# POSTECH-CVLab/InstaOrder

Hardware: AMD Instinct MI355X
Metric: instance-pairs/sec (fwd+bwd) (higher is better)
Workload: dtype f32

## Files before the change

instaorder_amd/csrc/conv_igemm.hip:

```cpp
#include <string.h>
#include <stdlib.h>

#include "io_common.h"

namespace {

constexpr int kThreads = 256;

__device__ __forceinline__ f32x4 ld4(const float* p) { return *reinterpret_cast<const f32x4*>(p); }
template <typename T> __device__ __forceinline__ void pin(T& v) { asm volatile("" : "+v"(v)); }
__device__ __forceinline__ void st4(float* p, f32x4 v) { *reinterpret_cast<f32x4*>(p) = v; }

__device__ __forceinline__ int xcd_remap(int b, int nwg) {
    const int q = nwg >> 3, r = nwg & 7, x = b & 7, i = b >> 3;
    return (x < r ? x * (q + 1) : r * (q + 1) + (x - r) * q) + i;
}

__device__ __forceinline__ int sdiv(int n, float rd) { return (int)(((float)n + 0.5f) * rd); }
__device__ __forceinline__ int stem_kp(int wT, int cr) { return (wT * cr + 31) / 32 * 32; }
__device__ __forceinline__ int fdiv(int n, IoFastDiv f) {
    return f.shift < 0 ? n : (int)(__umulhi((unsigned)n, f.magic) >> f.shift);
}

typedef unsigned u32x4 __attribute__((ext_vector_type(4)));
// ... 1958 lines not shown
        read_frags(0, na, nb);
        __builtin_amdgcn_sched_barrier(0);
        mma12(3, fa, fb);
#pragma unroll
        for (int j = 0; j < 3; ++j) { fa[j] = na[j]; fb[j] = nb[j]; }
    }
    if (kt0 < kt1) {
#pragma unroll
        for (int gi = 0; gi < 3; ++gi) {
            f32x4 na[3], nb[3];
            read_frags(gi + 1, na, nb);
            mma12(gi, fa, fb);
#pragma unroll
            for (int j = 0; j < 3; ++j) { fa[j] = na[j]; fb[j] = nb[j]; }
        }
        mma12(3, fa, fb);
    }

    const size_t wrow = (size_t)g.wT * g.Ci;
    float* base = dst + (size_t)split * g.Co * wrow + (size_t)(g.r0 + g.rs * fr) * g.S * g.Ci + c0 + wn * 32 + (lane & 31);
#pragma unroll
    for (int r = 0; r < 16; ++r) {
        const int o = o0 + wm * 32 + (r & 3) + 8 * (r >> 2) + 4 * (lane >> 5);
        const float s12 = acc[1][r] + acc[2][r], s34 = acc[3][r] + acc[4][r];
        float* p = base + (size_t)o * wrow;
        p[0] = 0.25f * acc[0][r] - (1.0f / 6.0f) * s12 + (1.0f / 24.0f) * s34;
        p[g.Ci] = (1.0f / 6.0f) * (acc[2][r] - acc[1][r]) + (1.0f / 12.0f) * (acc[3][r] - acc[4][r]);
        p[2 * g.Ci] = (1.0f / 6.0f) * (s34 - s12) + acc[5][r];
    }
}



template <bool BWE, bool XF, bool HALO = false>
__global__ __launch_bounds__(256, 2) void conv_wino4_kernel(IoConvGeom g, const float* __restrict__ in,
                                                        const float* __restrict__ U, float* __restrict__ out, int ntn,
                                                        size_t in_bytes, unsigned u_bytes, size_t out_bytes,
                                                        float* __restrict__ st_mean, float* __restrict__ st_m2,
                                                        IoBwStats bw) {
    constexpr int BM = 256, BN = 64, BK = 16, LDT = 16, NF = 6;
    constexpr int AQ = HALO ? 96 : 64;
    extern __shared__ __attribute__((aligned(16))) float smem[];
    float* sA = smem;
    float* sB = smem + NF * AQ * LDT;
    const int tid = threadIdx.x, lane = tid & 63;
    const int wave = __builtin_amdgcn_readfirstlane(tid >> 6);
    const int wm = wave >> 1, wn = wave & 1;
    const int tile = xcd_remap(blockIdx.x, gridDim.x);
    const int mt = tile / ntn;
    const int m0 = mt * BM, n0 = (tile - mt * ntn) * BN;
    const int HoWo = g.Ho * g.Wo;
    const int nkc = g.Ci / BK, nk = 3 * nkc;
    const int n_lo = fdiv(m0, g.fd_howo);
    const __amdgpu_buffer_rsrc_t rs_in = make_rsrc_at(in, (size_t)n_lo * (size_t)(g.Hi * g.Wi) * (size_t)(g.Ci * 4), in_bytes);
    const __amdgpu_buffer_rsrc_t rs_u = make_rsrc(U, u_bytes);

    const int sr = tid >> 2, sc = tid & 3;
    unsigned arow, urow;
    int aho;
    bool aleft, aright;
    constexpr int NI = HALO ? 2 : 1;
    const int Q = g.Wo >> 2;
    const int ns = HALO ? (HoWo >= BM ? 1 : BM / HoWo) : 1;
    const int RS = HALO ? (64 / Q) / ns : 1;
    const int HB = (RS + 2) * Q, hq_n = ns * HB;
    unsigned hrow[NI];
    bool hvalid[NI], hleft[NI], hright[NI];
    const bool has2 = HALO && 64 + sr < hq_n;
    const bool wave_has2 = HALO && 64 + wave * 16 < hq_n;
    if constexpr (HALO) {
        const int rem0 = m0 - n_lo * HoWo;
        const int h0 = ns > 1 ? 0 : fdiv(rem0, g.fd_wo);
#pragma unroll
        for (int it = 0; it < NI; ++it) {
            const int hq = sr + 64 * it;
            const int sm = hq / HB, hl = hq - sm * HB;
            const int hr = hl / Q, cq = hl - hr * Q;
            const int hi = h0 - 1 + hr, wo = 4 * cq;
            hvalid[it] = (it == 0 || has2) && (unsigned)hi < (unsigned)g.Hi;
            hleft[it] = wo > 0;
            hright[it] = wo + 4 < g.Wi;
            hrow[it] = (unsigned)((((sm * g.Hi + hi) * g.Wi + wo) * g.Ci + sc * 4) * 4);
        }
        aho = 0; aleft = aright = false; arow = 0;
        urow = (unsigned)((n0 + sr) * g.Ci + sc * 4) * 4u;
    } else {
        const int m = m0 + 4 * sr;
        const int n = fdiv(m, g.fd_howo), rem = m - n * HoWo;
        const int ho = fdiv(rem, g.fd_wo), wo = rem - ho * g.Wo;
        aho = ho;
        aleft = wo > 0;
        aright = wo + 4 < g.Wi;
        arow = (unsigned)((((n - n_lo) * g.Hi + ho) * g.Wi + wo) * g.Ci + sc * 4) * 4u;
        urow = (unsigned)((n0 + sr) * g.Ci + sc * 4) * 4u;
    }
    const unsigned uplane = (unsigned)(g.Co * g.Ci) * 4u;
    const int xgrp = XF ? m0 / bw.in_Mg : 0;
    const __amdgpu_buffer_rsrc_t rs_xs = make_rsrc(XF ? (const void*)(bw.in_scale + (size_t)xgrp * g.Ci) : (const void*)U,
                                                   XF ? (unsigned)g.Ci * 4u : 0u);
    const __amdgpu_buffer_rsrc_t rs_xh = make_rsrc(XF ? (const void*)(bw.in_shift + (size_t)xgrp * g.Ci) : (const void*)U,
                                                   XF ? (unsigned)g.Ci * 4u : 0u);
    const __amdgpu_buffer_rsrc_t rs_xm = make_rsrc((XF && bw.in_mean) ? (const void*)(bw.in_mean + (size_t)xgrp * g.Ci)
                                                                      : (const void*)U,
                                                   (XF && bw.in_mean) ? (unsigned)g.Ci * 4u : 0u);
    f32x4 pa[6], pu[6], xm, xs, xh;
    f32x4 pa2[HALO ? 6 : 1];
    unsigned xok = 0, xok2 = 0;
    int th = 0, cc = 0;
    auto load_tile = [&]() {
        const unsigned uoff = (unsigned)(th * NF) * uplane + (unsigned)(cc * BK) * 4u;
        if constexpr (HALO) {
#pragma unroll
            for (int f = 0; f < NF; ++f) pu[f] = bld4(rs_u, urow + uoff + (unsigned)f * uplane);
            if (th != 0) return;
            if constexpr (XF) {
                const unsigned coff = (unsigned)(cc * BK + sc * 4) * 4u;
                xm = bld4(rs_xm, coff);
                xs = bld4(rs_xs, coff);
                xh = bld4(rs_xh, coff);
            }
            const unsigned aoff = (unsigned)((cc * BK - g.Ci) * 4);
            xok = xok2 = 0;
#pragma unroll
            for (int i = 0; i < 6; ++i) {
                const bool ok = hvalid[0] & (i == 0 ? hleft[0] : i == 5 ? hright[0] : true);
                xok |= ok ? (1u << i) : 0u;
                pa[i] = bld4(rs_in, ok ? hrow[0] + aoff + (unsigned)(i * g.Ci * 4) : kInvalidOff);
            }
            if (wave_has2) {
#pragma unroll
                for (int i = 0; i < 6; ++i) {
                    const bool ok = hvalid[NI - 1] & (i == 0 ? hleft[NI - 1] : i == 5 ? hright[NI - 1] : true);
                    xok2 |= ok ? (1u << i) : 0u;
                    pa2[i] = bld4(rs_in, ok ? hrow[NI - 1] + aoff + (unsigned)(i * g.Ci * 4) : kInvalidOff);
                }
            }
            return;
        }
        const int dh = g.dh0 + g.dhs * th;
        const unsigned aoff = (unsigned)(((dh * g.Wi - 1) * g.Ci + cc * BK) * 4);
        if constexpr (XF) {
            const unsigned coff = (unsigned)(cc * BK + sc * 4) * 4u;
            xm = bld4(rs_xm, coff);
            xs = bld4(rs_xs, coff);
            xh = bld4(rs_xh, coff);
        }
        const bool rowok = (unsigned)(aho + dh) < (unsigned)g.Hi;
        xok = 0;
#pragma unroll
        for (int i = 0; i < 6; ++i) {
            const bool ok = rowok & (i == 0 ? aleft : i == 5 ? aright : true);
            xok |= ok ? (1u << i) : 0u;
            pa[i] = bld4(rs_in, ok ? arow + aoff + (unsigned)(i * g.Ci * 4) : kInvalidOff);
        }
#pragma unroll
        for (int f = 0; f < NF; ++f) pu[f] = bld4(rs_u, urow + uoff + (unsigned)f * uplane);
    };
    auto advance = [&]() {
        if constexpr (HALO) {
            const bool wrap = th == 2;
            th = wrap ? 0 : th + 1;
            cc += wrap ? 1 : 0;
            return;
        }
        const int c1 = cc + 1;
        const bool wrap = c1 == nkc;
        cc = wrap ? 0 : c1;
        th += wrap ? 1 : 0;
    };
    auto xform_item = [&](f32x4 (&p)[6], unsigned okbits) {
        if constexpr (XF) {
#pragma unroll
            for (int i = 0; i < 6; ++i) {
                const bool ok = (okbits >> i) & 1u;
#pragma unroll
                for (int e = 0; e < 4; ++e) {
                    const float v = fmaxf(__builtin_fmaf(p[i][e] - xm[e], xs[e], xh[e]), 0.f);
                    p[i][e] = ok ? v : 0.f;
                }
            }
        }
        const f32x4 d0 = p[0], d1 = p[1], d2 = p[2], d3 = p[3], d4 = p[4], d5 = p[5];
        const f32x4 e42 = d4 - 4.f * d2, e31 = d3 - 4.f * d1, f42 = d4 - d2, f31 = d3 - d1;
        p[0] = 4.f * d0 - 5.f * d2 + d4;
        p[1] = e42 + e31;
        p[2] = e42 - e31;
        p[3] = f42 + 2.f * f31;
        p[4] = f42 - 2.f * f31;
        p[5] = 4.f * d1 - 5.f * d3 + d5;
    };
    auto xform_tile = [&]() {
        if constexpr (HALO) {
            if (th != 0) return;
            xform_item(pa, xok);
            if (wave_has2) xform_item(pa2, xok2);
            return;
        }
        xform_item(pa, xok);
    };
    const int swz = sc ^ ((sr >> 2) & 3);
    auto store_tile = [&]() {
        float* a = sA + sr * LDT + swz * 4;
        float* b = sB + sr * LDT + swz * 4;
        if constexpr (HALO) {
#pragma unroll
            for (int f = 0; f < NF; ++f) st4(b + f * 64 * LDT, pu[f]);
            if (th != 0) return;
#pragma unroll
            for (int f = 0; f < NF; ++f) st4(a + f * AQ * LDT, pa[f]);
            if (has2) {
#pragma unroll
                for (int f = 0; f < NF; ++f) st4(a + (f * AQ + 64) * LDT, pa2[f]);
            }
            return;
        }
#pragma unroll
        for (int f = 0; f < NF; ++f) {
            st4(a + f * 64 * LDT, pa[f]);
            st4(b + f * 64 * LDT, pu[f]);
        }
    };

    f32x16 acc[NF];
#pragma unroll
    for (int f = 0; f < NF; ++f)
#pragma unroll
        for (int r = 0; r < 16; ++r) acc[f][r] = 0.f;

    const int frow = lane & 31;
    const int b_base = (wn * 32 + frow) * LDT;
    const int fsw = (frow >> 2) & 3;
    int arow_cur = wm * 32 + frow;
    const int arow_lane = HALO ? (wm * 32 + frow) + ((wm * 32 + frow) / (RS * Q)) * 2 * Q : 0;
    auto set_hoff = [&](int thc) {
        if constexpr (HALO) arow_cur = arow_lane + (1 + g.dh0 + g.dhs * thc) * Q;
    };
    auto read_frags = [&](int gi, f32x4 (&a)[3], f32x4 (&b)[3]) {
        const int cl = (gi >> 1) * 2 + (lane >> 5);
        const int chunk = cl ^ fsw;
        const int chunk_a = HALO ? (cl ^ ((arow_cur >> 2) & 3)) : chunk;
        const int f0 = (gi & 1) * 3;
#pragma unroll
        for (int j = 0; j < 3; ++j) {
            a[j] = ld4(sA + ((f0 + j) * AQ + arow_cur) * LDT + chunk_a * 4);
            b[j] = ld4(sB + (f0 + j) * 64 * LDT + b_base + chunk * 4);
        }
    };
    auto mma12 = [&](int gi, const f32x4 (&a)[3], const f32x4 (&b)[3]) {
        const int f0 = (gi & 1) * 3;
#pragma unroll
        for (int tt = 0; tt < 4; ++tt)
#pragma unroll
            for (int j = 0; j < 3; ++j)
                acc[f0 + j] = __builtin_amdgcn_mfma_f32_32x32x2f32(a[j][tt], b[j][tt], acc[f0 + j], 0, 0, 0);
    };

    f32x4 fa[3], fb[3];
    load_tile();
    xform_tile();
    store_tile();
    __syncthreads();
    int thc = 0;
    set_hoff(0);
    read_frags(0, fa, fb);
    for (int kt = 0; kt + 1 < nk; ++kt) {
        advance();
#pragma unroll
        for (int gi = 0; gi < 3; ++gi) {
            f32x4 na[3], nb[3];
            read_frags(gi + 1, na, nb);
            mma12(gi, fa, fb);
#pragma unroll
            for (int j = 0; j < 3; ++j) { fa[j] = na[j]; fb[j] = nb[j]; }
            if (gi == 0) {
                load_tile();
                __builtin_amdgcn_sched_barrier(0);
            }
            if (gi == 1) xform_tile();
        }
        __builtin_amdgcn_sched_barrier(0);
#pragma unroll
        for (int j = 0; j < 3; ++j) { pin(fa[j]); pin(fb[j]); }
        __syncthreads();
        store_tile();
        __syncthreads();
        thc = thc == 2 ? 0 : thc + 1;
        set_hoff(thc);
        f32x4 na[3], nb[3];
        read_frags(0, na, nb);
        __builtin_amdgcn_sched_barrier(0);
        mma12(3, fa, fb);
#pragma unroll
        for (int j = 0; j < 3; ++j) { fa[j] = na[j]; fb[j] = nb[j]; }
    }
#pragma unroll
    for (int gi = 0; gi < 3; ++gi) {
        f32x4 na[3], nb[3];
        read_frags(gi + 1, na, nb);
        mma12(gi, fa, fb);
#pragma unroll
        for (int j = 0; j < 3; ++j) { fa[j] = na[j]; fb[j] = nb[j]; }
    }
    mma12(3, fa, fb);

#pragma unroll
    for (int r = 0; r < 16; ++r) {
        const float s12 = acc[1][r] + acc[2][r], d12 = acc[1][r] - acc[2][r];
        const float s34 = acc[3][r] + acc[4][r], d34 = acc[3][r] - acc[4][r];
        const float y0 = acc[0][r] + s12 + s34, y3 = d12 + 8.f * d34 + acc[5][r];
        acc[1][r] = d12 + 2.f * d34;
        acc[2][r] = s12 + 4.f * s34;
        acc[0][r] = y0;
        acc[3][r] = y3;
    }
    const int st = 2 * mt + wm;
    const int co = n0 + wn * 32 + (lane & 31);
    if (st_mean) {
        float sum = 0.f;
#pragma unroll
        for (int i = 0; i < 4; ++i)
#pragma unroll
            for (int r = 0; r < 16; ++r) sum += acc[i][r];
        sum += __shfl_xor(sum, 32, 64);
        const float mean = sum * (1.0f / 128.0f);
        float m2 = 0.f;
#pragma unroll
        for (int i = 0; i < 4; ++i)
#pragma unroll
            for (int r = 0; r < 16; ++r) m2 += (acc[i][r] - mean) * (acc[i][r] - mean);
        m2 += __shfl_xor(m2, 32, 64);
        if (lane < 32) {
            st_mean[(size_t)st * g.Co + co] = mean;
            st_m2[(size_t)st * g.Co + co] = m2;
        }
    }
    const size_t out_base = (size_t)(m0 + wm * 128) * (size_t)(g.Co * 4);
// ... 20 lines not shown
                const float t = __builtin_fmaf(yv[r] - mu, sc_, sh_);
                float v = acc[i][r];
                if (bw.mscale) v = t > 0.f ? v : 0.f;
                s1 += v;
                s2 += v * ((yv[r] - mu) * rs);
                st_el_s<float>(v, rs_out, lane_off, so);
                st_el_s<float>(fmaxf(t, 0.f), rs_ao, lane_off, so);
            }
        }
        s1 += __shfl_xor(s1, 32, 64);
        s2 += __shfl_xor(s2, 32, 64);
        if (lane < 32) {
            bw.p1[(size_t)st * g.Co + co] = s1;
            bw.p2[(size_t)st * g.Co + co] = s2;
        }
    } else {
        const float bias = bw.bias ? bw.bias[co] : 0.f;
#pragma unroll
        for (int i = 0; i < 4; ++i)
#pragma unroll
            for (int r = 0; r < 16; ++r) {
                float v = acc[i][r];
                if (bw.bias) {
                    v += bias;
                    v = (bw.relu && v < 0.f) ? 0.f : v;
                }
                st_el_s<float>(v, rs_out, lane_off, (unsigned)(4 * ((r & 3) + 8 * (r >> 2)) + i) * rowstep);
            }
    }
}

__global__ __launch_bounds__(256) void wino4_filter_kernel(const float* __restrict__ w, float* __restrict__ U, int Co,
                                                          int Ci, int S, int r0, int rs, int s0, int ss, int dw0,
                                                          int dws) {
    const int th = blockIdx.y, c4n = Ci / 4;
    const int idx = blockIdx.x * 256 + threadIdx.x;
    if (idx >= Co * c4n) return;
    const int o = idx / c4n, c = (idx - o * c4n) * 4;
    f32x4 gq[3];
#pragma unroll
    for (int j = 0; j < 3; ++j) {
        const int tw = (j - 1 - dw0) * dws;
        const int tap = (r0 + rs * th) * S + s0 + ss * tw;
        gq[j] = ld4(w + ((size_t)o * (3 * S) + tap) * Ci + c);
    }
    const size_t plane = (size_t)Co * Ci;
    float* dst = U + (size_t)th * 6 * plane + (size_t)o * Ci + c;
    const f32x4 s02 = gq[0] + gq[2], q02 = gq[0] + 4.f * gq[2];
    st4(dst, 0.25f * gq[0]);
    st4(dst + plane, (-1.0f / 6.0f) * (s02 + gq[1]));
    st4(dst + 2 * plane, (-1.0f / 6.0f) * (s02 - gq[1]));
    st4(dst + 3 * plane, (1.0f / 24.0f) * (q02 + 2.f * gq[1]));
    st4(dst + 4 * plane, (1.0f / 24.0f) * (q02 - 2.f * gq[1]));
    st4(dst + 5 * plane, gq[2]);
}

__global__ __launch_bounds__(256) void wino_filter_kernel(const float* __restrict__ w, float* __restrict__ U, int Co,
                                                         int Ci, int S, int r0, int rs, int s0, int ss, int dw0,
                                                         int dws) {
    const int th = blockIdx.y, c4n = Ci / 4;
    const int idx = blockIdx.x * 256 + threadIdx.x;
    if (idx >= Co * c4n) return;
    const int o = idx / c4n, c = (idx - o * c4n) * 4;
    f32x4 gq[3];
#pragma unroll
    for (int j = 0; j < 3; ++j) {
        const int tw = (j - 1 - dw0) * dws;
        const int tap = (r0 + rs * th) * S + s0 + ss * tw;
        gq[j] = ld4(w + ((size_t)o * (3 * S) + tap) * Ci + c);
    }
    const size_t plane = (size_t)Co * Ci;
    float* dst = U + (size_t)th * 4 * plane + (size_t)o * Ci + c;
    st4(dst, gq[0]);
    st4(dst + plane, 0.5f * (gq[0] + gq[1] + gq[2]));
    st4(dst + 2 * plane, 0.5f * (gq[0] - gq[1] + gq[2]));
    st4(dst + 3 * plane, gq[2]);
}

__global__ __launch_bounds__(256) void splitk_reduce_kernel(const float* __restrict__ partial,
                                                           float* __restrict__ dst, size_t n4, int splits) {
    __shared__ f32x4 red[8][32];
    const int tx = threadIdx.x & 31, ty = threadIdx.x >> 5;
    const size_t i = (size_t)blockIdx.x * 32 + tx;
    const bool ok = i < n4;
    const f32x4* p4 = reinterpret_cast<const f32x4*>(partial);
    f32x4 s = {0.f, 0.f, 0.f, 0.f};
    if (ok)
// ... 44 lines not shown
        p.tiles = (g.Co / p.bmo) * g.Th * g.Tw * p.ntile_c;
    }
    if (p.tiles < 1) p.tiles = 1;
    const bool fp32_tr = fp32 && !stem && !g.gw && p.bmo == 128 && p.bnc == 128;
    const int nkt = io_cdiv(M, 32);
    int want = (fp32_tr ? (p.tiles >= 128 ? 2304 : 768) : 1024) / p.tiles;
    int maxs = nkt / 8 > 0 ? nkt / 8 : 1;
    p.splits = want < maxs ? want : maxs;
    if (p.splits < 1) p.splits = 1;
    p.kps = io_cdiv(nkt, p.splits);
    p.splits = io_cdiv(nkt, p.kps);
    return p;
}

bool wgrad_wino_shape_ok(const IoConvGeom& g, int stem) {
    return !stem && !g.gw && !g.cr && g.Th == 3 && g.Tw == 3 && g.S == 3 && g.wT == 9 && g.is == 1 &&
           g.os == 1 && g.Hi == g.Ho && g.Wi == g.Wo && g.dh0 == -1 && g.dhs == 1 && g.dw0 == -1 && g.dws == 1 &&
           g.rs == 1 && g.ss == 1 && g.r0 == 0 && g.s0 == 0 && g.Wo % 8 == 0 && ((long)g.N * g.Ho * g.Wo) % 64 == 0 &&
           g.Ci % 64 == 0 && g.Co % 64 == 0;
}
bool wgrad_wino_ok(const IoConvGeom& g, int stem) { return io_wino_on() && wgrad_wino_shape_ok(g, stem); }
WgradPlan plan_wgrad_wino(const IoConvGeom& g) {
    WgradPlan p;
    p.bmo = p.bnc = 64;
    p.ntile_c = g.Ci / 64;
    p.tiles = (g.Co / 64) * 3 * p.ntile_c;
    const int nkt = (int)(((long)g.N * g.Ho * g.Wo) / 64);
    const int want = 1024 / p.tiles, maxs = nkt / 8 > 0 ? nkt / 8 : 1;
    p.splits = want < maxs ? want : maxs;
    if (p.splits < 1) p.splits = 1;
    p.kps = io_cdiv(nkt, p.splits);
    p.splits = io_cdiv(nkt, p.kps);
    return p;
}

}

size_t io_conv_wgrad_partial_bytes(const IoConvGeom& g, int stem) {
    const int s0 = plan_wgrad(g, stem, true).splits, s1 = plan_wgrad(g, stem, false).splits;
    int splits = s0 > s1 ? s0 : s1;
    if (wgrad_wino_shape_ok(g, stem)) {
        const int sw = plan_wgrad_wino(g).splits;
        if (sw > splits) splits = sw;
    }
    size_t need = splits == 1 ? 0 : (size_t)splits * g.Co * io_filter_row(g) * sizeof(float);
    if (stem && g.cr && io_stem_rows_ok(g)) {
        const size_t rows = (size_t)io_stem_wgrad_rows_max_blocks() * g.Co * io_filter_row(g) * sizeof(float);
        if (rows > need) need = rows;
    }
    if (stem && !g.cr && g.Ci == 8 && g.Co == 64 && g.Wo == 128)
        if (io_stem_wgrad_halo_partial_bytes() > need) need = io_stem_wgrad_halo_partial_bytes();
    if (!stem && io_wgrad_halo3_shape(g) && io_wgrad_halo3_partial_bytes() > need) need = io_wgrad_halo3_partial_bytes();
    return need;
}

static std::atomic<int> g_last_wgrad_route{0};
extern "C" int io_debug_last_wgrad_route(void) { return g_last_wgrad_route.load(std::memory_order_relaxed); }
static std::atomic<int> g_last_route{0};
extern "C" int io_debug_last_nt_route(void) { return g_last_route.load(std::memory_order_relaxed); }

int io_launch_conv_nt(const IoConvGeom& g, const void* in, const void* wgt, void* out, const void* add,
                      const void* mask, int stem, hipStream_t st, float* st_mean, float* st_m2,
                      const IoBwStats* bw, int dt_in, int dt_out) {
    IoBwStats bws;
    memset(&bws, 0, sizeof(bws));
    if (bw) {
// ... 68 lines not shown
    static std::atomic<int> small_tiles_c{-1};
    int small_tiles = small_tiles_c.load(std::memory_order_relaxed);
    if (small_tiles < 0) {
        const char* e = getenv("IO_NT_SMALL_TILES");
        small_tiles = e ? atoi(e) : 256;
        small_tiles_c.store(small_tiles, std::memory_order_relaxed);
    }
    const long tiles128 = (long)io_cdiv(M, 128) * (g.Co / 128);
    const int bn = g.gw ? g.gw : ((g.Co % 128 == 0 && tiles128 > small_tiles) ? 128 : 64);
    IO_REQUIRE(!g.gw || (g.gw == 64 && !stem && g.Ci == g.Co), IO_ERR_SHAPE,
               "conv_nt: grouped mode needs a 64-channel window and Ci == Co");
    const int ntn = g.Co / bn;
    const long tiles = (long)io_cdiv(M, 128) * ntn;
    IO_REQUIRE(tiles < (1L << 31), IO_ERR_SHAPE, "conv_nt: grid too large");
    dim3 grid((unsigned)tiles), block(kThreads);
    const bool lin = !stem && !g.gw && g.Th * g.Tw == 1 && g.is == 1 && g.os == 1 && g.dh0 == 0 && g.dw0 == 0 &&
                     g.Hi == g.Ho && g.Wi == g.Wo && g.outH == g.Ho && g.outW == g.Wo && M % 128 == 0 &&
                     128.0 * g.Ci * es < 4.0e9 && 128.0 * g.Co * os < 4.0e9;
    IO_REQUIRE(!bws.xb_res || lin, IO_ERR_SHAPE, "conv_nt: the residual operand form needs a dense 1x1 stride-1 GEMM on whole tiles");
    if (io_wino_on() && bws.wino_u && !stem && !g.gw && dt_in == IO_F32 && dt_out == IO_F32 && g.Th == 3 && g.Tw == 3 &&
        g.S == 3 && g.wT == 9 && g.is == 1 && g.os == 1 && g.Hi == g.Ho && g.Wi == g.Wo && g.outH == g.Ho &&
        g.outW == g.Wo && g.Wo % 2 == 0 && M % 128 == 0 && g.Ci % 32 == 0 && !add && !mask && !bws.xb_a &&
        g.dhs * g.dhs == 1 && g.dws * g.dws == 1 && g.dw0 * (g.dw0 + 2 * g.dws) == -1 && g.rs == 1 && g.ss == 1 &&
        !(bws.y && bws.in_scale) && 12.0 * g.Co * g.Ci * 4.0 < 4.0e9) {
        const double kred9 = 9.0 * g.Ci;
        const bool wino4 = g.Wo % 4 == 0 && M % 256 == 0 && g.Ci % 16 == 0 && (!bws.y || bws.Mg % 256 == 0) &&
                           (!bws.in_scale || bws.in_Mg % 256 == 0) && 18.0 * g.Co * g.Ci * 4.0 < 4.0e9;
        const double fl9 = 2.0 * (double)M * g.Co * kred9;
        IoProfScope prof(IO_PROF_CONV_WINO, fl9,
                         (double)os * M * g.Co * (1.0 + (bws.y ? 1.0 : 0.0)) +
                             (double)es * ((double)g.N * g.Hi * g.Wi * g.Ci + (double)g.Co * kred9), st,
                         wino4 ? fl9 * 0.5 : fl9 * (2.0 / 3.0));
        if (wino4) {
            hipLaunchKernelGGL(wino4_filter_kernel, dim3((unsigned)io_cdiv((long)g.Co * g.Ci / 4, 256), 3), dim3(256), 0, st,
                               (const float*)wgt, bws.wino_u, g.Co, g.Ci, g.S, g.r0, g.rs, g.s0, g.ss, g.dw0, g.dws);
            const unsigned u_bytes = (unsigned)(18.0 * g.Co * g.Ci * 4.0);
            const int ntw = g.Co / 64;
            dim3 grid4((unsigned)((M / 256) * ntw));
            const long hw = (long)g.Ho * g.Wo;
            const bool halo = g.Wo <= 64 && 256 % g.Wo == 0 &&
                              (hw % 256 == 0 || (256 % hw == 0 && (256 / hw) * (g.Ho + 2) * (g.Wo / 4) <= 96));
            const size_t lds4 = (size_t)6 * ((halo ? 96 : 64) + 64) * 16 * sizeof(float);
#define IO_LAUNCH_W4_(BWE_, XF_, HALO_)                                                                                 \
    hipLaunchKernelGGL((conv_wino4_kernel<BWE_, XF_, HALO_>), grid4, block, lds4, st, g, (const float*)in,              \
                       (const float*)bws.wino_u, (float*)out, ntw, in_bytes, u_bytes, out_bytes, st_mean, st_m2, bws)
            if (halo) {
                if (bws.y) IO_LAUNCH_W4_(true, false, true);
                else if (bws.in_scale) IO_LAUNCH_W4_(false, true, true);
                else IO_LAUNCH_W4_(false, false, true);
            } else {
                if (bws.y) IO_LAUNCH_W4_(true, false, false);
                else if (bws.in_scale) IO_LAUNCH_W4_(false, true, false);
                else IO_LAUNCH_W4_(false, false, false);
            }
#undef IO_LAUNCH_W4_
            return io_check_launch("conv_nt(wino4)");
        }
        hipLaunchKernelGGL(wino_filter_kernel, dim3((unsigned)io_cdiv((long)g.Co * g.Ci / 4, 256), 3), dim3(256), 0, st,
                           (const float*)wgt, bws.wino_u, g.Co, g.Ci, g.S, g.r0, g.rs, g.s0, g.ss, g.dw0, g.dws);
        const unsigned wu_bytes = (unsigned)(12.0 * g.Co * g.Ci * 4.0);
        const int ntw = g.Co / 64;
        dim3 gridw((unsigned)((M / 128) * ntw));
        const size_t ldsz = (size_t)(256 + 256) * 32 * sizeof(float);
#define IO_LAUNCH_WINO_(BWE_, XF_)                                                                                    \
    do {                                                                                                             \
        static std::atomic<unsigned long long> attr_done{0};                                                         \
        if (io_first_on_device(attr_done))                                                                           \
            (void)hipFuncSetAttribute(                                                                               \
                (const void*)conv_nt_kernel<float, float, 64, 0, 4, 1, 2, BWE_, XF_, false, 0, true>,                \
                hipFuncAttributeMaxDynamicSharedMemorySize, (int)ldsz);                                              \
        hipLaunchKernelGGL((conv_nt_kernel<float, float, 64, 0, 4, 1, 2, BWE_, XF_, false, 0, true>), gridw, block,  \
                           ldsz, st, g, (const float*)in, (const float*)bws.wino_u, (float*)out, (const float*)nullptr, \
                           (const float*)nullptr, ntw, in_bytes, wu_bytes, out_bytes, st_mean, st_m2, bws);          \
    } while (0)
        if (bws.y) IO_LAUNCH_WINO_(true, false);
        else if (bws.in_scale) IO_LAUNCH_WINO_(false, true);
        else IO_LAUNCH_WINO_(false, false);
#undef IO_LAUNCH_WINO_
// ... 276 lines not shown
```

Measured before the change: 1760.

## Stream Winograd filter fragments directly from global memory in MFMA layout

The wino4 filter transform now writes U in a fragment-major layout that matches the MFMA B-operand lane order. The conv kernel loads B fragments straight from global memory into registers with buffer loads and prefetches them one group ahead, instead of staging them through LDS. LDS is now used only for the A (input transform) tile, which is double-buffered in the halo variant so it needs fewer barriers. This removes the LDS traffic and synchronisation for B, at the cost of more global/L2 loads per wave and more register pressure. The LDS size is changed accordingly, and the max dynamic shared memory attribute is set on first launch.

```diff
diff --git a/instaorder_amd/csrc/conv_igemm.hip b/instaorder_amd/csrc/conv_igemm.hip
--- a/instaorder_amd/csrc/conv_igemm.hip
+++ b/instaorder_amd/csrc/conv_igemm.hip
@@ -2014,6 +2014,12 @@
 
 
 
+__host__ __device__ inline unsigned wino4_u_index(int th, int f, int o, int c, int Co, int Ci) {
+    const int cc = c >> 4, cl = (c >> 2) & 3;
+    return (unsigned)((((th * (Ci >> 4) + cc) * (Co >> 5) + (o >> 5)) * 6 + f) * 2 + (cl >> 1)) * 256u +
+           (unsigned)(((cl & 1) * 32 + (o & 31)) * 4 + (c & 3));
+}
+
 template <bool BWE, bool XF, bool HALO = false>
 __global__ __launch_bounds__(256, 2) void conv_wino4_kernel(IoConvGeom g, const float* __restrict__ in,
                                                         const float* __restrict__ U, float* __restrict__ out, int ntn,
@@ -2022,9 +2028,9 @@
                                                         IoBwStats bw) {
     constexpr int BM = 256, BN = 64, BK = 16, LDT = 16, NF = 6;
     constexpr int AQ = HALO ? 96 : 64;
+    constexpr int ABUF = NF * AQ * LDT;
     extern __shared__ __attribute__((aligned(16))) float smem[];
     float* sA = smem;
-    float* sB = smem + NF * AQ * LDT;
     const int tid = threadIdx.x, lane = tid & 63;
     const int wave = __builtin_amdgcn_readfirstlane(tid >> 6);
     const int wm = wave >> 1, wn = wave & 1;
@@ -2038,7 +2044,7 @@
     const __amdgpu_buffer_rsrc_t rs_u = make_rsrc(U, u_bytes);
 
     const int sr = tid >> 2, sc = tid & 3;
-    unsigned arow, urow;
+    unsigned arow;
     int aho;
     bool aleft, aright;
     constexpr int NI = HALO ? 2 : 1;
@@ -2065,7 +2071,6 @@
             hrow[it] = (unsigned)((((sm * g.Hi + hi) * g.Wi + wo) * g.Ci + sc * 4) * 4);
         }
         aho = 0; aleft = aright = false; arow = 0;
-        urow = (unsigned)((n0 + sr) * g.Ci + sc * 4) * 4u;
     } else {
         const int m = m0 + 4 * sr;
         const int n = fdiv(m, g.fd_howo), rem = m - n * HoWo;
@@ -2074,9 +2079,7 @@
         aleft = wo > 0;
         aright = wo + 4 < g.Wi;
         arow = (unsigned)((((n - n_lo) * g.Hi + ho) * g.Wi + wo) * g.Ci + sc * 4) * 4u;
-        urow = (unsigned)((n0 + sr) * g.Ci + sc * 4) * 4u;
-    }
-    const unsigned uplane = (unsigned)(g.Co * g.Ci) * 4u;
+    }
     const int xgrp = XF ? m0 / bw.in_Mg : 0;
     const __amdgpu_buffer_rsrc_t rs_xs = make_rsrc(XF ? (const void*)(bw.in_scale + (size_t)xgrp * g.Ci) : (const void*)U,
                                                    XF ? (unsigned)g.Ci * 4u : 0u);
@@ -2085,22 +2088,17 @@
     const __amdgpu_buffer_rsrc_t rs_xm = make_rsrc((XF && bw.in_mean) ? (const void*)(bw.in_mean + (size_t)xgrp * g.Ci)
                                                                       : (const void*)U,
                                                    (XF && bw.in_mean) ? (unsigned)g.Ci * 4u : 0u);
-    f32x4 pa[6], pu[6], xm, xs, xh;
+    f32x4 pa[6], xm, xs, xh;
     f32x4 pa2[HALO ? 6 : 1];
     unsigned xok = 0, xok2 = 0;
-    int th = 0, cc = 0;
-    auto load_tile = [&]() {
-        const unsigned uoff = (unsigned)(th * NF) * uplane + (unsigned)(cc * BK) * 4u;
+    auto load_a = [&](int th, int cc) {
+        if constexpr (XF) {
+            const unsigned coff = (unsigned)(cc * BK + sc * 4) * 4u;
+            xm = bld4(rs_xm, coff);
+            xs = bld4(rs_xs, coff);
+            xh = bld4(rs_xh, coff);
+        }
         if constexpr (HALO) {
-#pragma unroll
-            for (int f = 0; f < NF; ++f) pu[f] = bld4(rs_u, urow + uoff + (unsigned)f * uplane);
-            if (th != 0) return;
-            if constexpr (XF) {
-                const unsigned coff = (unsigned)(cc * BK + sc * 4) * 4u;
-                xm = bld4(rs_xm, coff);
-                xs = bld4(rs_xs, coff);
-                xh = bld4(rs_xh, coff);
-            }
             const unsigned aoff = (unsigned)((cc * BK - g.Ci) * 4);
             xok = xok2 = 0;
 #pragma unroll
@@ -2121,12 +2119,6 @@
         }
         const int dh = g.dh0 + g.dhs * th;
         const unsigned aoff = (unsigned)(((dh * g.Wi - 1) * g.Ci + cc * BK) * 4);
-        if constexpr (XF) {
-            const unsigned coff = (unsigned)(cc * BK + sc * 4) * 4u;
-            xm = bld4(rs_xm, coff);
-            xs = bld4(rs_xs, coff);
-            xh = bld4(rs_xh, coff);
-        }
         const bool rowok = (unsigned)(aho + dh) < (unsigned)g.Hi;
         xok = 0;
 #pragma unroll
@@ -2135,20 +2127,6 @@
             xok |= ok ? (1u << i) : 0u;
             pa[i] = bld4(rs_in, ok ? arow + aoff + (unsigned)(i * g.Ci * 4) : kInvalidOff);
         }
-#pragma unroll
-        for (int f = 0; f < NF; ++f) pu[f] = bld4(rs_u, urow + uoff + (unsigned)f * uplane);
-    };
-    auto advance = [&]() {
-        if constexpr (HALO) {
-            const bool wrap = th == 2;
-            th = wrap ? 0 : th + 1;
-            cc += wrap ? 1 : 0;
-            return;
-        }
-        const int c1 = cc + 1;
-        const bool wrap = c1 == nkc;
-        cc = wrap ? 0 : c1;
-        th += wrap ? 1 : 0;
     };
     auto xform_item = [&](f32x4 (&p)[6], unsigned okbits) {
         if constexpr (XF) {
@@ -2171,36 +2149,21 @@
         p[4] = f42 - 2.f * f31;
         p[5] = 4.f * d1 - 5.f * d3 + d5;
     };
-    auto xform_tile = [&]() {
-        if constexpr (HALO) {
-            if (th != 0) return;
-            xform_item(pa, xok);
+    auto xform_a = [&]() {
+        xform_item(pa, xok);
+        if constexpr (HALO)
             if (wave_has2) xform_item(pa2, xok2);
-            return;
-        }
-        xform_item(pa, xok);
     };
     const int swz = sc ^ ((sr >> 2) & 3);
-    auto store_tile = [&]() {
-        float* a = sA + sr * LDT + swz * 4;
-        float* b = sB + sr * LDT + swz * 4;
-        if constexpr (HALO) {
-#pragma unroll
-            for (int f = 0; f < NF; ++f) st4(b + f * 64 * LDT, pu[f]);
-            if (th != 0) return;
-#pragma unroll
-            for (int f = 0; f < NF; ++f) st4(a + f * AQ * LDT, pa[f]);
+    auto store_a = [&](int buf) {
+        float* a = sA + buf * ABUF + sr * LDT + swz * 4;
+#pragma unroll
+        for (int f = 0; f < NF; ++f) st4(a + f * AQ * LDT, pa[f]);
+        if constexpr (HALO)
             if (has2) {
 #pragma unroll
                 for (int f = 0; f < NF; ++f) st4(a + (f * AQ + 64) * LDT, pa2[f]);
             }
-            return;
-        }
-#pragma unroll
-        for (int f = 0; f < NF; ++f) {
-            st4(a + f * 64 * LDT, pa[f]);
-            st4(b + f * 64 * LDT, pu[f]);
-        }
     };
 
     f32x16 acc[NF];
@@ -2210,23 +2173,30 @@
         for (int r = 0; r < 16; ++r) acc[f][r] = 0.f;
 
     const int frow = lane & 31;
-    const int b_base = (wn * 32 + frow) * LDT;
-    const int fsw = (frow >> 2) & 3;
     int arow_cur = wm * 32 + frow;
     const int arow_lane = HALO ? (wm * 32 + frow) + ((wm * 32 + frow) / (RS * Q)) * 2 * Q : 0;
     auto set_hoff = [&](int thc) {
         if constexpr (HALO) arow_cur = arow_lane + (1 + g.dh0 + g.dhs * thc) * Q;
     };
-    auto read_frags = [&](int gi, f32x4 (&a)[3], f32x4 (&b)[3]) {
+    int abuf = 0;
+    auto read_a = [&](int gi, f32x4 (&a)[3]) {
         const int cl = (gi >> 1) * 2 + (lane >> 5);
-        const int chunk = cl ^ fsw;
-        const int chunk_a = HALO ? (cl ^ ((arow_cur >> 2) & 3)) : chunk;
+        const int chunk_a = cl ^ ((arow_cur >> 2) & 3);
         const int f0 = (gi & 1) * 3;
 #pragma unroll
-        for (int j = 0; j < 3; ++j) {
-            a[j] = ld4(sA + ((f0 + j) * AQ + arow_cur) * LDT + chunk_a * 4);
-            b[j] = ld4(sB + (f0 + j) * 64 * LDT + b_base + chunk * 4);
-        }
+        for (int j = 0; j < 3; ++j) a[j] = ld4(sA + abuf * ABUF + ((f0 + j) * AQ + arow_cur) * LDT + chunk_a * 4);
+    };
+    const int ncb = g.Co >> 5, cb = (n0 >> 5) + wn;
+    const unsigned ulane = (unsigned)lane * 16u;
+    auto ubase = [&](int k) -> unsigned {
+        k = k < nk ? k : nk - 1;
+        const int kth = HALO ? k % 3 : k / nkc, kcc = HALO ? k / 3 : k - kth * nkc;
+        return (unsigned)(((kth * nkc + kcc) * ncb + cb) * 12288);
+    };
+    auto load_b = [&](unsigned base, int gi, f32x4 (&b)[3]) {
+        const int f0 = (gi & 1) * 3, kk = gi >> 1;
+#pragma unroll
+        for (int j = 0; j < 3; ++j) b[j] = bld4(rs_u, ulane + base + (unsigned)(((f0 + j) * 2 + kk) * 1024));
     };
     auto mma12 = [&](int gi, const f32x4 (&a)[3], const f32x4 (&b)[3]) {
         const int f0 = (gi & 1) * 3;
@@ -2237,53 +2207,76 @@
                 acc[f0 + j] = __builtin_amdgcn_mfma_f32_32x32x2f32(a[j][tt], b[j][tt], acc[f0 + j], 0, 0, 0);
     };
 
-    f32x4 fa[3], fb[3];
-    load_tile();
-    xform_tile();
-    store_tile();
+    f32x4 fa[3], b0[3], b1[3];
+    unsigned ub = ubase(0), ubn = ubase(1);
+    load_b(ub, 0, b0);
+    load_b(ub, 1, b1);
+    load_a(0, 0);
+    xform_a();
+    store_a(0);
     __syncthreads();
-    int thc = 0;
+    int thc = 0, ccm = 0;
     set_hoff(0);
-    read_frags(0, fa, fb);
-    for (int kt = 0; kt + 1 < nk; ++kt) {
-        advance();
+    read_a(0, fa);
+    for (int kt = 0; kt < nk; ++kt) {
+        const bool more = kt + 1 < nk;
+        const bool next_v = HALO && ccm + 1 < nkc;
 #pragma unroll
         for (int gi = 0; gi < 3; ++gi) {
             f32x4 na[3], nb[3];
-            read_frags(gi + 1, na, nb);
-            mma12(gi, fa, fb);
-#pragma unroll
-            for (int j = 0; j < 3; ++j) { fa[j] = na[j]; fb[j] = nb[j]; }
-            if (gi == 0) {
-                load_tile();
-                __builtin_amdgcn_sched_barrier(0);
-            }
-            if (gi == 1) xform_tile();
+            read_a(gi + 1, na);
+            load_b(gi < 2 ? ub : ubn, (gi + 2) & 3, nb);
+            mma12(gi, fa, b0);
+#pragma unroll
+            for (int j = 0; j < 3; ++j) { fa[j] = na[j]; b0[j] = b1[j]; b1[j] = nb[j]; }
+            if constexpr (HALO) {
+                if (gi == 0 && thc == 0 && next_v) {
+                    load_a(0, ccm + 1);
+                    __builtin_amdgcn_sched_barrier(0);
+                }
+                if (gi == 2 && thc == 0 && next_v) {
+                    xform_a();
+                    store_a(abuf ^ 1);
+                }
+            } else {
+                if (gi == 0 && more) {
+                    const int c1 = ccm + 1 == nkc ? 0 : ccm + 1;
+                    load_a(c1 == 0 ? thc + 1 : thc, c1);
+                    __builtin_amdgcn_sched_barrier(0);
+                }
+                if (gi == 1 && more) xform_a();
+            }
         }
         __builtin_amdgcn_sched_barrier(0);
-#pragma unroll
-        for (int j = 0; j < 3; ++j) { pin(fa[j]); pin(fb[j]); }
-        __syncthreads();
-        store_tile();
-        __syncthreads();
-        thc = thc == 2 ? 0 : thc + 1;
+        if constexpr (HALO) {
+            if (thc == 2) {
+#pragma unroll
+                for (int j = 0; j < 3; ++j) pin(fa[j]);
+                __syncthreads();
+                abuf ^= 1;
+                ++ccm;
+            }
+            thc = thc == 2 ? 0 : thc + 1;
+        } else if (more) {
+#pragma unroll
+            for (int j = 0; j < 3; ++j) pin(fa[j]);
+            __syncthreads();
+            store_a(0);
+            __syncthreads();
+            ++ccm;
+            if (ccm == nkc) { ccm = 0; ++thc; }
+        }
         set_hoff(thc);
         f32x4 na[3], nb[3];
-        read_frags(0, na, nb);
+        read_a(0, na);
+        load_b(ubn, 1, nb);
         __builtin_amdgcn_sched_barrier(0);
-        mma12(3, fa, fb);
-#pragma unroll
-        for (int j = 0; j < 3; ++j) { fa[j] = na[j]; fb[j] = nb[j]; }
-    }
-#pragma unroll
-    for (int gi = 0; gi < 3; ++gi) {
-        f32x4 na[3], nb[3];
-        read_frags(gi + 1, na, nb);
-        mma12(gi, fa, fb);
-#pragma unroll
-        for (int j = 0; j < 3; ++j) { fa[j] = na[j]; fb[j] = nb[j]; }
-    }
-    mma12(3, fa, fb);
+        mma12(3, fa, b0);
+#pragma unroll
+        for (int j = 0; j < 3; ++j) { fa[j] = na[j]; b0[j] = b1[j]; b1[j] = nb[j]; }
+        ub = ubn;
+        ubn = ubase(kt + 2);
+    }
 
 #pragma unroll
     for (int r = 0; r < 16; ++r) {
@@ -2382,15 +2375,14 @@
         const int tap = (r0 + rs * th) * S + s0 + ss * tw;
         gq[j] = ld4(w + ((size_t)o * (3 * S) + tap) * Ci + c);
     }
-    const size_t plane = (size_t)Co * Ci;
-    float* dst = U + (size_t)th * 6 * plane + (size_t)o * Ci + c;
+    float* dst = U + wino4_u_index(th, 0, o, c, Co, Ci);
     const f32x4 s02 = gq[0] + gq[2], q02 = gq[0] + 4.f * gq[2];
     st4(dst, 0.25f * gq[0]);
-    st4(dst + plane, (-1.0f / 6.0f) * (s02 + gq[1]));
-    st4(dst + 2 * plane, (-1.0f / 6.0f) * (s02 - gq[1]));
-    st4(dst + 3 * plane, (1.0f / 24.0f) * (q02 + 2.f * gq[1]));
-    st4(dst + 4 * plane, (1.0f / 24.0f) * (q02 - 2.f * gq[1]));
-    st4(dst + 5 * plane, gq[2]);
+    st4(dst + 512, (-1.0f / 6.0f) * (s02 + gq[1]));
+    st4(dst + 2 * 512, (-1.0f / 6.0f) * (s02 - gq[1]));
+    st4(dst + 3 * 512, (1.0f / 24.0f) * (q02 + 2.f * gq[1]));
+    st4(dst + 4 * 512, (1.0f / 24.0f) * (q02 - 2.f * gq[1]));
+    st4(dst + 5 * 512, gq[2]);
 }
 
 __global__ __launch_bounds__(256) void wino_filter_kernel(const float* __restrict__ w, float* __restrict__ U, int Co,
@@ -2643,10 +2635,16 @@
             const long hw = (long)g.Ho * g.Wo;
             const bool halo = g.Wo <= 64 && 256 % g.Wo == 0 &&
                               (hw % 256 == 0 || (256 % hw == 0 && (256 / hw) * (g.Ho + 2) * (g.Wo / 4) <= 96));
-            const size_t lds4 = (size_t)6 * ((halo ? 96 : 64) + 64) * 16 * sizeof(float);
+            const size_t lds4 = (size_t)6 * (halo ? 2 * 96 : 64) * 16 * sizeof(float);
 #define IO_LAUNCH_W4_(BWE_, XF_, HALO_)                                                                                 \
-    hipLaunchKernelGGL((conv_wino4_kernel<BWE_, XF_, HALO_>), grid4, block, lds4, st, g, (const float*)in,              \
-                       (const float*)bws.wino_u, (float*)out, ntw, in_bytes, u_bytes, out_bytes, st_mean, st_m2, bws)
+    do {                                                                                                             \
+        static std::atomic<unsigned long long> attr_done{0};                                                         \
+        if (io_first_on_device(attr_done))                                                                           \
+            (void)hipFuncSetAttribute((const void*)conv_wino4_kernel<BWE_, XF_, HALO_>,                              \
+                                      hipFuncAttributeMaxDynamicSharedMemorySize, (int)lds4);                        \
+        hipLaunchKernelGGL((conv_wino4_kernel<BWE_, XF_, HALO_>), grid4, block, lds4, st, g, (const float*)in,          \
+                           (const float*)bws.wino_u, (float*)out, ntw, in_bytes, u_bytes, out_bytes, st_mean, st_m2, bws); \
+    } while (0)
             if (halo) {
                 if (bws.y) IO_LAUNCH_W4_(true, false, true);
                 else if (bws.in_scale) IO_LAUNCH_W4_(false, true, true);
```

Result: no change. 1762 (median of 6 runs) (+0.1%).

## Load Winograd filter fragments directly from L2 in MFMA layout, bypassing LDS

Applied to the files above, without the earlier changes.

The filter transform kernel can now write U in a fragment-major layout that matches the MFMA B-operand lanes. The wino4 conv kernel then loads B fragments straight from global/L2 with buffer loads, two groups ahead, instead of staging them through LDS. It restructures the main loop so that per stage only the A tile goes through LDS. This cuts LDS footprint and LDS traffic, which may allow more occupancy, at the cost of more global load latency and register pressure. The path is on by default and can be turned off with an environment variable.

```diff
diff --git a/instaorder_amd/csrc/conv_igemm.hip b/instaorder_amd/csrc/conv_igemm.hip
--- a/instaorder_amd/csrc/conv_igemm.hip
+++ b/instaorder_amd/csrc/conv_igemm.hip
@@ -2014,7 +2014,7 @@
 
 
 
-template <bool BWE, bool XF, bool HALO = false>
+template <bool BWE, bool XF, bool HALO = false, bool UL2 = false>
 __global__ __launch_bounds__(256, 2) void conv_wino4_kernel(IoConvGeom g, const float* __restrict__ in,
                                                         const float* __restrict__ U, float* __restrict__ out, int ntn,
                                                         size_t in_bytes, unsigned u_bytes, size_t out_bytes,
@@ -2092,8 +2092,10 @@
     auto load_tile = [&]() {
         const unsigned uoff = (unsigned)(th * NF) * uplane + (unsigned)(cc * BK) * 4u;
         if constexpr (HALO) {
-#pragma unroll
-            for (int f = 0; f < NF; ++f) pu[f] = bld4(rs_u, urow + uoff + (unsigned)f * uplane);
+            if constexpr (!UL2) {
+#pragma unroll
+                for (int f = 0; f < NF; ++f) pu[f] = bld4(rs_u, urow + uoff + (unsigned)f * uplane);
+            }
             if (th != 0) return;
             if constexpr (XF) {
                 const unsigned coff = (unsigned)(cc * BK + sc * 4) * 4u;
@@ -2135,10 +2137,16 @@
             xok |= ok ? (1u << i) : 0u;
             pa[i] = bld4(rs_in, ok ? arow + aoff + (unsigned)(i * g.Ci * 4) : kInvalidOff);
         }
-#pragma unroll
-        for (int f = 0; f < NF; ++f) pu[f] = bld4(rs_u, urow + uoff + (unsigned)f * uplane);
+        if constexpr (!UL2) {
+#pragma unroll
+            for (int f = 0; f < NF; ++f) pu[f] = bld4(rs_u, urow + uoff + (unsigned)f * uplane);
+        }
     };
     auto advance = [&]() {
+        if constexpr (HALO && UL2) {
+            ++cc;
+            return;
+        }
         if constexpr (HALO) {
             const bool wrap = th == 2;
             th = wrap ? 0 : th + 1;
@@ -2185,8 +2193,10 @@
         float* a = sA + sr * LDT + swz * 4;
         float* b = sB + sr * LDT + swz * 4;
         if constexpr (HALO) {
-#pragma unroll
-            for (int f = 0; f < NF; ++f) st4(b + f * 64 * LDT, pu[f]);
+            if constexpr (!UL2) {
+#pragma unroll
+                for (int f = 0; f < NF; ++f) st4(b + f * 64 * LDT, pu[f]);
+            }
             if (th != 0) return;
 #pragma unroll
             for (int f = 0; f < NF; ++f) st4(a + f * AQ * LDT, pa[f]);
@@ -2199,7 +2209,7 @@
 #pragma unroll
         for (int f = 0; f < NF; ++f) {
             st4(a + f * 64 * LDT, pa[f]);
-            st4(b + f * 64 * LDT, pu[f]);
+            if constexpr (!UL2) st4(b + f * 64 * LDT, pu[f]);
         }
     };
 
@@ -2237,16 +2247,121 @@
                 acc[f0 + j] = __builtin_amdgcn_mfma_f32_32x32x2f32(a[j][tt], b[j][tt], acc[f0 + j], 0, 0, 0);
     };
 
-    f32x4 fa[3], fb[3];
-    load_tile();
-    xform_tile();
-    store_tile();
-    __syncthreads();
-    int thc = 0;
-    set_hoff(0);
-    read_frags(0, fa, fb);
-    for (int kt = 0; kt + 1 < nk; ++kt) {
-        advance();
+    if constexpr (UL2) {
+        constexpr int TPS = HALO ? 3 : 1, GPS = 4 * TPS;
+        const int nstage = HALO ? nkc : nk;
+        const unsigned ulane = (unsigned)(((n0 >> 5) + wn) * (g.Ci >> 3)) * 1024u + (unsigned)lane * 16u;
+        int bth = 0, bcc = 0;
+        auto fetch_b = [&](int gi, f32x4 (&b)[3]) {
+            const unsigned soff = (unsigned)(bth * NF + (gi & 1) * 3) * uplane + (unsigned)(bcc * 2 + (gi >> 1)) * 1024u;
+#pragma unroll
+            for (int j = 0; j < 3; ++j)
+                b[j] = __builtin_bit_cast(f32x4, __builtin_amdgcn_raw_buffer_load_b128(rs_u, ulane, soff + (unsigned)j * uplane, 0));
+            if (gi == 3) {
+                if constexpr (HALO) {
+                    const bool wrap = bth == 2;
+                    bth = wrap ? 0 : bth + 1;
+                    bcc += wrap ? 1 : 0;
+                } else {
+                    const bool wrap = bcc + 1 == nkc;
+                    bcc = wrap ? 0 : bcc + 1;
+                    bth += wrap ? 1 : 0;
+                }
+            }
+        };
+        auto read_a = [&](int gi, f32x4 (&a)[3]) {
+            const int cl = (gi >> 1) * 2 + (lane >> 5);
+            const int chunk_a = HALO ? (cl ^ ((arow_cur >> 2) & 3)) : (cl ^ fsw);
+            const int f0 = (gi & 1) * 3;
+#pragma unroll
+            for (int j = 0; j < 3; ++j) a[j] = ld4(sA + ((f0 + j) * AQ + arow_cur) * LDT + chunk_a * 4);
+        };
+        f32x4 fa[3], fb[3], nb[3];
+        load_tile();
+        fetch_b(0, fb);
+        fetch_b(1, nb);
+        xform_tile();
+        store_tile();
+        __syncthreads();
+        set_hoff(0);
+        read_a(0, fa);
+        for (int s = 0; s < nstage; ++s) {
+            const bool more = s + 1 < nstage;
+#pragma unroll
+            for (int q = 0; q < GPS; ++q) {
+                const int gi = q & 3;
+                f32x4 nnb[3], na[3];
+                if (q + 2 < GPS || more) fetch_b((q + 2) & 3, nnb);
+                if (q + 1 < GPS) {
+                    if (gi == 3) set_hoff((q + 1) >> 2);
+                    read_a((q + 1) & 3, na);
+                }
+                if (q == 0 && more) {
+                    advance();
+                    load_tile();
+                    __builtin_amdgcn_sched_barrier(0);
+                }
+                if (q == (HALO ? 3 : 1) && more) xform_tile();
+                if (q + 1 == GPS && more) {
+                    __builtin_amdgcn_sched_barrier(0);
+#pragma unroll
+                    for (int j = 0; j < 3; ++j) pin(fa[j]);
+                    __syncthreads();
+                    store_tile();
+                    __syncthreads();
+                    set_hoff(0);
+                    read_a(0, na);
+                    __builtin_amdgcn_sched_barrier(0);
+                }
+                mma12(gi, fa, fb);
+#pragma unroll
+                for (int j = 0; j < 3; ++j) {
+                    fa[j] = na[j];
+                    fb[j] = nb[j];
+                    nb[j] = nnb[j];
+                }
+                __builtin_amdgcn_sched_barrier(0);
+            }
+        }
+    } else {
+        f32x4 fa[3], fb[3];
+        load_tile();
+        xform_tile();
+        store_tile();
+        __syncthreads();
+        int thc = 0;
+        set_hoff(0);
+        read_frags(0, fa, fb);
+        for (int kt = 0; kt + 1 < nk; ++kt) {
+            advance();
+#pragma unroll
+            for (int gi = 0; gi < 3; ++gi) {
+                f32x4 na[3], nb[3];
+                read_frags(gi + 1, na, nb);
+                mma12(gi, fa, fb);
+#pragma unroll
+                for (int j = 0; j < 3; ++j) { fa[j] = na[j]; fb[j] = nb[j]; }
+                if (gi == 0) {
+                    load_tile();
+                    __builtin_amdgcn_sched_barrier(0);
+                }
+                if (gi == 1) xform_tile();
+            }
+            __builtin_amdgcn_sched_barrier(0);
+#pragma unroll
+            for (int j = 0; j < 3; ++j) { pin(fa[j]); pin(fb[j]); }
+            __syncthreads();
+            store_tile();
+            __syncthreads();
+            thc = thc == 2 ? 0 : thc + 1;
+            set_hoff(thc);
+            f32x4 na[3], nb[3];
+            read_frags(0, na, nb);
+            __builtin_amdgcn_sched_barrier(0);
+            mma12(3, fa, fb);
+#pragma unroll
+            for (int j = 0; j < 3; ++j) { fa[j] = na[j]; fb[j] = nb[j]; }
+        }
 #pragma unroll
         for (int gi = 0; gi < 3; ++gi) {
             f32x4 na[3], nb[3];
@@ -2254,36 +2369,9 @@
             mma12(gi, fa, fb);
 #pragma unroll
             for (int j = 0; j < 3; ++j) { fa[j] = na[j]; fb[j] = nb[j]; }
-            if (gi == 0) {
-                load_tile();
-                __builtin_amdgcn_sched_barrier(0);
-            }
-            if (gi == 1) xform_tile();
-        }
-        __builtin_amdgcn_sched_barrier(0);
-#pragma unroll
-        for (int j = 0; j < 3; ++j) { pin(fa[j]); pin(fb[j]); }
-        __syncthreads();
-        store_tile();
-        __syncthreads();
-        thc = thc == 2 ? 0 : thc + 1;
-        set_hoff(thc);
-        f32x4 na[3], nb[3];
-        read_frags(0, na, nb);
-        __builtin_amdgcn_sched_barrier(0);
+        }
         mma12(3, fa, fb);
-#pragma unroll
-        for (int j = 0; j < 3; ++j) { fa[j] = na[j]; fb[j] = nb[j]; }
-    }
-#pragma unroll
-    for (int gi = 0; gi < 3; ++gi) {
-        f32x4 na[3], nb[3];
-        read_frags(gi + 1, na, nb);
-        mma12(gi, fa, fb);
-#pragma unroll
-        for (int j = 0; j < 3; ++j) { fa[j] = na[j]; fb[j] = nb[j]; }
-    }
-    mma12(3, fa, fb);
+    }
 
 #pragma unroll
     for (int r = 0; r < 16; ++r) {
@@ -2370,7 +2458,7 @@
 
 __global__ __launch_bounds__(256) void wino4_filter_kernel(const float* __restrict__ w, float* __restrict__ U, int Co,
                                                           int Ci, int S, int r0, int rs, int s0, int ss, int dw0,
-                                                          int dws) {
+                                                          int dws, int frag) {
     const int th = blockIdx.y, c4n = Ci / 4;
     const int idx = blockIdx.x * 256 + threadIdx.x;
     if (idx >= Co * c4n) return;
@@ -2383,7 +2471,9 @@
         gq[j] = ld4(w + ((size_t)o * (3 * S) + tap) * Ci + c);
     }
     const size_t plane = (size_t)Co * Ci;
-    float* dst = U + (size_t)th * 6 * plane + (size_t)o * Ci + c;
+    const size_t pos = frag ? ((size_t)((o >> 5) * (Ci >> 3) + (c >> 3)) * 64 + ((c >> 2) & 1) * 32 + (o & 31)) * 4
+                            : (size_t)o * Ci + c;
+    float* dst = U + (size_t)th * 6 * plane + pos;
     const f32x4 s02 = gq[0] + gq[2], q02 = gq[0] + 4.f * gq[2];
     st4(dst, 0.25f * gq[0]);
     st4(dst + plane, (-1.0f / 6.0f) * (s02 + gq[1]));
@@ -2501,6 +2591,17 @@
     p.kps = io_cdiv(nkt, p.splits);
     p.splits = io_cdiv(nkt, p.kps);
     return p;
+}
+
+std::atomic<int> g_wino4_form{-1};
+int wino4_form() {
+    int v = g_wino4_form.load(std::memory_order_relaxed);
+    if (v < 0) {
+        const char* e = getenv("IO_WINO4_FORM");
+        v = (e && e[0] == '0') ? 0 : 1;
+        g_wino4_form.store(v, std::memory_order_relaxed);
+    }
+    return v;
 }
 
 }
@@ -2635,18 +2736,27 @@
                              (double)es * ((double)g.N * g.Hi * g.Wi * g.Ci + (double)g.Co * kred9), st,
                          wino4 ? fl9 * 0.5 : fl9 * (2.0 / 3.0));
         if (wino4) {
+            const int ul2 = wino4_form();
             hipLaunchKernelGGL(wino4_filter_kernel, dim3((unsigned)io_cdiv((long)g.Co * g.Ci / 4, 256), 3), dim3(256), 0, st,
-                               (const float*)wgt, bws.wino_u, g.Co, g.Ci, g.S, g.r0, g.rs, g.s0, g.ss, g.dw0, g.dws);
+                               (const float*)wgt, bws.wino_u, g.Co, g.Ci, g.S, g.r0, g.rs, g.s0, g.ss, g.dw0, g.dws, ul2);
             const unsigned u_bytes = (unsigned)(18.0 * g.Co * g.Ci * 4.0);
             const int ntw = g.Co / 64;
             dim3 grid4((unsigned)((M / 256) * ntw));
             const long hw = (long)g.Ho * g.Wo;
             const bool halo = g.Wo <= 64 && 256 % g.Wo == 0 &&
                               (hw % 256 == 0 || (256 % hw == 0 && (256 / hw) * (g.Ho + 2) * (g.Wo / 4) <= 96));
-            const size_t lds4 = (size_t)6 * ((halo ? 96 : 64) + 64) * 16 * sizeof(float);
+            const size_t lds4 = (size_t)6 * ((halo ? 96 : 64) + (ul2 ? 0 : 64)) * 16 * sizeof(float);
 #define IO_LAUNCH_W4_(BWE_, XF_, HALO_)                                                                                 \
-    hipLaunchKernelGGL((conv_wino4_kernel<BWE_, XF_, HALO_>), grid4, block, lds4, st, g, (const float*)in,              \
-                       (const float*)bws.wino_u, (float*)out, ntw, in_bytes, u_bytes, out_bytes, st_mean, st_m2, bws)
+    do {                                                                                                                \
+        if (ul2)                                                                                                        \
+            hipLaunchKernelGGL((conv_wino4_kernel<BWE_, XF_, HALO_, true>), grid4, block, lds4, st, g,                  \
+                               (const float*)in, (const float*)bws.wino_u, (float*)out, ntw, in_bytes, u_bytes,         \
+                               out_bytes, st_mean, st_m2, bws);                                                         \
+        else                                                                                                            \
+            hipLaunchKernelGGL((conv_wino4_kernel<BWE_, XF_, HALO_, false>), grid4, block, lds4, st, g,                 \
+                               (const float*)in, (const float*)bws.wino_u, (float*)out, ntw, in_bytes, u_bytes,         \
+                               out_bytes, st_mean, st_m2, bws);                                                         \
+    } while (0)
             if (halo) {
                 if (bws.y) IO_LAUNCH_W4_(true, false, true);
                 else if (bws.in_scale) IO_LAUNCH_W4_(false, true, true);
```

New measurement: 1813 before, 1825 after (median of 6 runs). No clear change (+0.7%).
